# MIMUW-RL/space-gym

Measured on AMD Instinct MI355X. Metric: env-steps/sec at batch=65536, GoalContinuous3P-v0, 1/2/4/8 MI355X, higher is better.
Workload: dtype f32

## Files before the change

include/spacegym.h:

```cpp
#ifndef SPACEGYM_H
#define SPACEGYM_H

#include <stddef.h>
#include <stdint.h>

#ifdef __cplusplus
extern "C" {
#endif

#define SG_OK 0
#define SG_ERR_INVALID -1
#define SG_ERR_HIP -2
#define SG_ERR_NO_DEVICE -3

typedef struct sg_env sg_env;

typedef struct sg_config {
    char env_id[64];
    int64_t num_envs;
    uint64_t seed;
    uint32_t env_index_base;
    int32_t max_episode_steps;
    int32_t auto_reset;
    int32_t steering;
// ... 318 lines not shown
    int32_t activation;
    float log_std_min;
    float log_std_max;
    sg_policy_mlp actor;
    int32_t reserved;
} sg_squashed_policy;
int sg_squashed_act_device(sg_env *env, const sg_squashed_policy *sp, const float *obs_dev, uint64_t seed, uint64_t step,
                           int32_t deterministic, float *action_out, float *logp_out, void *hip_stream);
int sg_squashed_sample_device(sg_env *env, const sg_squashed_policy *sp, int64_t n, const float *obs, const float *eps,
                              float *action_out, float *logp_out, void *hip_stream);
typedef struct sg_squashed_grads {
    uint32_t struct_size;
    uint32_t reserved;
    sg_policy_grads_mlp actor;
} sg_squashed_grads;
int sg_squashed_grad_device(sg_env *env, const sg_squashed_policy *sp, int64_t n, const float *obs, const float *eps,
                            const float *g_action, const float *g_logp, const sg_squashed_grads *grads, void *workspace,
                            size_t workspace_bytes, void *hip_stream);
size_t sg_squashed_grad_workspace_bytes(sg_env *env, const sg_squashed_policy *sp, int64_t n);
int sg_rollout_squashed_device(sg_env *env, int32_t n_steps, const sg_squashed_policy *sp, uint64_t seed, uint64_t first_step,
                               int32_t deterministic, float *obs, float *action, float *logp, float *reward, uint8_t *done,
                               uint8_t *truncated, const sg_terminal_list *terminal_list, void *hip_stream);

int sg_vector_field(sg_env *env, const void *actions_host, const float *ship_host, float *out_host);

void *sg_host_alloc(size_t bytes);
void sg_host_free(void *ptr);

int sg_set_profiling(sg_env *env, int32_t on);
int sg_get_profile(sg_env *env, int64_t *launches, double *total_ms, double *min_ms, double *max_ms);

const char *sg_rollout_kernel(sg_env *env, int32_t n_steps);

void *sg_stream(const sg_env *env);

const char *sg_version(void);

#ifdef __cplusplus
}
#endif
#endif
```

space_gym_amd/_native.py:

```python
import ctypes as C
import os

_HERE = os.path.dirname(os.path.abspath(__file__))
LIB_PATH = os.environ.get("SPACEGYM_LIB") or os.path.join(_HERE, "lib", "libspacegym_hip.so")
_lib = None


class SgConfig(C.Structure):
    _fields_ = [("env_id", C.c_char * 64), ("num_envs", C.c_int64), ("seed", C.c_uint64),
                ("env_index_base", C.c_uint32), ("max_episode_steps", C.c_int32), ("auto_reset", C.c_int32),
                ("steering", C.c_int32)]


class SgParams(C.Structure):
    _fields_ = [("struct_size", C.c_uint32), ("n_planets", C.c_int32), ("randomize", C.c_int32), ("reserved", C.c_int32),
                ("goal_vel_reward_scale", C.c_double), ("safety_reward_scale", C.c_double), ("goal_sparse_reward", C.c_double),
                ("survival_reward_scale", C.c_double), ("danger_zone", C.c_double),
                ("ref_orbit_a", C.c_double), ("ref_orbit_eccentricity", C.c_double), ("ref_orbit_angle", C.c_double),
                ("numerator_C", C.c_double), ("rad_penalty_C", C.c_double), ("act_penalty_C", C.c_double), ("step_size", C.c_double),
                ("ship_moi", C.c_double), ("max_engine_force", C.c_double)]


class SgTerminalList(C.Structure):
    _fields_ = [("count", C.c_void_p), ("step_env", C.c_void_p), ("obs", C.c_void_p), ("capacity", C.c_uint32)]
# ... 167 lines not shown
    "sg_priority_begin_device": (C.c_int, [_vp, C.POINTER(SgPriority), _vp]),
    "sg_priority_commit_device": (C.c_int, [_vp, C.POINTER(SgPriority), C.c_int32, C.c_int32, C.c_int32, _vp]),
    "sg_priority_update_device": (C.c_int, [_vp, C.POINTER(SgPriority), C.c_int64, _vp, _vp, _vp]),
    "sg_priority_sample_config_init": (None, [C.POINTER(SgPrioritySampleConfig)]),
    "sg_priority_sample_device": (C.c_int, [_vp, C.POINTER(SgReplay), C.POINTER(SgPriority), C.POINTER(SgPrioritySampleConfig), C.c_int64,
                                            C.POINTER(SgPriorityDraw), _vp]),
    "sg_policy_act_device": (C.c_int, [_vp, C.POINTER(SgPolicy), _vp, C.c_uint64, C.c_uint64, C.c_int32, _vp, _vp, _vp, _vp]),
    "sg_rollout_policy_device": (C.c_int, [_vp, C.c_int32, C.POINTER(SgPolicy), C.c_uint64, C.c_uint64, C.c_int32, _vp, _vp, _vp, _vp,
                                           _vp, _vp, _vp, C.POINTER(SgTerminalList), _vp, _vp]),
    "sg_policy_evaluate_device": (C.c_int, [_vp, C.POINTER(SgPolicy), C.c_int64, _vp, _vp, _vp, _vp, _vp, _vp]),
    "sg_policy_grad_device": (C.c_int, [_vp, C.POINTER(SgPolicy), C.c_int64, _vp, _vp, _vp, _vp, _vp, C.POINTER(SgPolicyGrads), _vp, C.c_size_t, _vp]),
    "sg_policy_grad_workspace_bytes": (C.c_size_t, [_vp, C.POINTER(SgPolicy), C.c_int64]),
    "sg_q_evaluate_device": (C.c_int, [_vp, C.POINTER(SgQnet), C.c_int64, _vp, _vp, _vp, _vp, _vp]),
    "sg_q_grad_device": (C.c_int, [_vp, C.POINTER(SgQnet), C.c_int64, _vp, _vp, _vp, _vp, C.POINTER(SgQnetGrads), _vp, _vp, C.c_size_t, _vp]),
    "sg_q_grad_workspace_bytes": (C.c_size_t, [_vp, C.POINTER(SgQnet), C.c_int64]),
    "sg_policy_action_device": (C.c_int, [_vp, C.POINTER(SgPolicy), C.c_int64, _vp, _vp, _vp, _vp]),
    "sg_policy_action_grad_device": (C.c_int, [_vp, C.POINTER(SgPolicy), C.c_int64, _vp, _vp, _vp, C.POINTER(SgPolicyGrads), _vp, C.c_size_t, _vp]),
    "sg_squashed_act_device": (C.c_int, [_vp, C.POINTER(SgSquashedPolicy), _vp, C.c_uint64, C.c_uint64, C.c_int32, _vp, _vp, _vp]),
    "sg_squashed_sample_device": (C.c_int, [_vp, C.POINTER(SgSquashedPolicy), C.c_int64, _vp, _vp, _vp, _vp, _vp]),
    "sg_squashed_grad_device": (C.c_int, [_vp, C.POINTER(SgSquashedPolicy), C.c_int64, _vp, _vp, _vp, _vp, C.POINTER(SgSquashedGrads), _vp,
                                          C.c_size_t, _vp]),
    "sg_squashed_grad_workspace_bytes": (C.c_size_t, [_vp, C.POINTER(SgSquashedPolicy), C.c_int64]),
    "sg_rollout_squashed_device": (C.c_int, [_vp, C.c_int32, C.POINTER(SgSquashedPolicy), C.c_uint64, C.c_uint64, C.c_int32, _vp, _vp, _vp, _vp,
                                             _vp, _vp, C.POINTER(SgTerminalList), _vp]),
    "sg_get_state": (C.c_int, [_vp, _vp, _vp, _vp, _vp]),
    "sg_set_state": (C.c_int, [_vp, _vp, _vp, _vp, _vp]),
    "sg_vector_field": (C.c_int, [_vp, _vp, _vp, _vp]),
    "sg_host_alloc": (_vp, [C.c_size_t]),
    "sg_host_free": (None, [_vp]),
    "sg_set_profiling": (C.c_int, [_vp, C.c_int32]),
    "sg_get_profile": (C.c_int, [_vp, C.POINTER(C.c_int64), C.POINTER(C.c_double), C.POINTER(C.c_double), C.POINTER(C.c_double)]),
    "sg_stream": (_vp, [_vp]),
    "sg_rollout_kernel": (C.c_char_p, [_vp, C.c_int32]),
    "sg_random_actions_device": (C.c_int, [_vp, C.c_int32, C.c_uint64, C.c_uint64, _vp, _vp]),
    "sg_version": (C.c_char_p, []),
}


def load():
    global _lib
    if _lib is not None:
        return _lib
    if not os.path.exists(LIB_PATH):
        raise NativeError(f"{LIB_PATH} not found: build it with `python -m space_gym_amd.build` "
                          "(hipcc, gfx950). The engine is HIP-only; there is no CPU fallback.")
    try:
        import torch
    except ImportError:
        pass
    lib = C.CDLL(LIB_PATH)
    for name, (res, args) in SYMBOLS.items():
        try:
            fn = getattr(lib, name)
        except AttributeError:
            if not os.environ.get("SPACEGYM_LIB"):
                raise
            continue
        fn.restype, fn.argtypes = res, args
    _lib = lib
    return lib


def check(lib, handle, rc, what):
    if rc != 0:
        msg = lib.sg_last_error(handle)
        raise NativeError(f"{what} failed ({rc}): {msg.decode() if msg else ''}")
# ... 1 lines not shown
```

space_gym_amd/csrc/sg_engine.hip:

```cpp
#include <hip/hip_runtime.h>
#include <hip/hip_ext.h>

#include <algorithm>
#include <cmath>
#include <cstdarg>
#include <cstdio>
#include <cstdlib>
#include <cstring>
#include <limits>
#include <new>
#include <string>
#include <tuple>
#include <type_traits>
#include <utility>
#include <vector>

#include "../../include/spacegym.h"

#ifdef SG_STAMPS
constexpr int kStampSlots = 16, kStampWaves = 4096;
__device__ unsigned long long sg_dbg_stamps[kStampSlots * kStampWaves];
#ifdef SG_STAMPS_ACC_ONLY
#define SG_STAMP(slot)
#else
// ... 1076 lines not shown
    constexpr int D = 7 + 2 * N + 2;
    const bool have = (uint32_t)lane < n;
    const uint32_t slot = (lo + (have ? (uint32_t)lane : 0u)) % (uint32_t)kReplayCap;
    uint32_t step_lane;
    GoalEnv<N> e;
    float2 a;
    GoalReplay<N>::get(rb, slot, step_lane, e, a);
    double dXd, dYd;
    GoalReplay<N>::get_result(rb, slot, dXd, dYd);
    int hit;
    float rew;
    if constexpr (RS::kOn) rew = goal_reward<N>(rs.goal(c, wave_env0 + (int)(step_lane & 63u)), e.x, e.y, dXd, dYd, e.px, e.py, e.gx, e.gy, hit);
    else rew = goal_reward<N>(c, e.x, e.y, dXd, dYd, e.px, e.py, e.gx, e.gy, hit);
    count_hits(cnt, have && hit);
    const int t = (int)(step_lane >> 6), env = wave_env0 + (int)(step_lane & 63u);
    if (have) reward[(int64_t)t * B + env] = rew;
    if constexpr (TOBS) {
        e.x = (float)((double)e.x + dXd); e.y = (float)((double)e.y + dYd);
        float o[D];
        goal_observe<N>(c, e, o);
        term_append<D>(tl, have, t, env, o);
    }
}

template <int N, bool ACCEL, int kSpare, bool TOBS>
__global__ __launch_bounds__(kPairBlock) void goal_pair_rollout_kernel(const SgDev *__restrict__ cfg, const SgBuffers *__restrict__ bufs,
                                                                    int num_envs, int n_steps,
                                                                    const void *__restrict__ actions, float *__restrict__ obs,
                                                                    float *__restrict__ reward, uint8_t *__restrict__ done,
                                                                    uint8_t *__restrict__ truncated,
                                                                    typename std::conditional<TOBS, TermList, NoTermList>::type tl,
                                                                    int *__restrict__ status) {
#define SG_ROLLOUT_PROFILED 0
#define SG_ROLLOUT_RS
#include "sg_goal_pair_rollout.inc"
#undef SG_ROLLOUT_RS
#undef SG_ROLLOUT_PROFILED
}
template <int N, bool ACCEL, int kSpare, bool TOBS>
__global__ __launch_bounds__(kPairBlock) void goal_pair_rollout_profiled_kernel(const SgDev *__restrict__ cfg,
                                                                             const SgBuffers *__restrict__ bufs, int num_envs, int n_steps,
                                                                             const void *__restrict__ actions, float *__restrict__ obs,
                                                                             float *__restrict__ reward, uint8_t *__restrict__ done,
                                                                             uint8_t *__restrict__ truncated,
                                                                             typename std::conditional<TOBS, TermList, NoTermList>::type tl,
                                                                             int *__restrict__ status, ProfileSource rs) {
#define SG_ROLLOUT_PROFILED 1
#define SG_ROLLOUT_RS , rs
#include "sg_goal_pair_rollout.inc"
#undef SG_ROLLOUT_RS
#undef SG_ROLLOUT_PROFILED
}

template <typename F, typename... X>
__device__ __forceinline__ void pair_step(const SgDev *cfg, SgBuffers b, int num_envs, const void *actions, float *obs,
                                          float *reward, uint8_t *done, uint8_t *truncated, float *terminal_obs, X... extra) {
    __shared__ float hand[kHand * kBlock];
    const int tid = threadIdx.x & (kBlock - 1);
    const bool pilot = threadIdx.x < kBlock;
    const int i = blockIdx.x * kBlock + tid;
    const bool live = i < num_envs;
    const int ii = live ? i : 0;
    typename F::Env e;
    F::load_env(b, ii, e);
    const SgDev &c = *cfg;
    if constexpr (F::kTouchParams) {
        const uint32_t *cw = reinterpret_cast<const uint32_t *>(cfg);
        uint32_t touch = 0u;
#pragma unroll
        for (int k = 0; k < (int)(sizeof(SgDev) / 4); k += 16) touch ^= cw[k];
        touch ^= cw[sizeof(SgDev) / 4 - 1];
        asm volatile("" ::"s"(touch));
    }
    const bool discrete = c.discrete_actions != 0;
    float2 a = make_float2(0.0f, 0.0f);
    if constexpr (F::kFinishAction) load_action(discrete, actions, ii, a.x, a.y);
    float *q = hand + tid;
    if (pilot) {
        if constexpr (!F::kFinishAction) load_action(discrete, actions, ii, a.x, a.y);
        StepResult r;
        F::integrate(c, e, a, r);
        const uint64_t ux = __double_as_longlong(r.dXd), uy = __double_as_longlong(r.dYd);
        q[0 * kBlock] = __uint_as_float((uint32_t)ux); q[1 * kBlock] = __uint_as_float((uint32_t)(ux >> 32));
// ... 1569 lines not shown
    __attribute__((always_inline)) sg_env() = default;
    SgDev dev = {};
    SgDev *d_cfg = nullptr;
    SgBuffers buf = {};
    SgBuffers *d_buf = nullptr;
    int device = 0;
    int fresh = 0;
    hipStream_t stream = nullptr;
    float *d_actions = nullptr, *d_obs = nullptr, *d_reward = nullptr, *d_tobs = nullptr, *d_ship = nullptr, *d_planets = nullptr, *d_goal = nullptr;
    uint8_t *d_done = nullptr, *d_trunc = nullptr;
    int32_t *d_elapsed = nullptr;
    int *h_status = nullptr, *d_status = nullptr;
    uint8_t *d_pack = nullptr, *h_pack[2] = {};
    uint8_t *h_pack_dev[2] = {};
    int host_out = 0;
    size_t pack_bytes = 0, pack_tobs = 0, pack_reward = 0, pack_done = 0, pack_trunc = 0;
    hipEvent_t step_event = nullptr;
    int pack_cur = 0, step_pending = 0, step_tobs = 0;
    double *d_ep_ret = nullptr, *d_epo_ret = nullptr;
    int32_t *d_ep_len = nullptr, *d_epo_len = nullptr;
    size_t pack_base_bytes = 0, pack_ep_ret = 0, pack_ep_len = 0;
    int step_eps = 0;
    int last_end = -1;
    sg_normalize norm = {};
    double *d_nstate = nullptr, *d_returns = nullptr, *d_npart = nullptr, *d_nmtab = nullptr, *d_nstab = nullptr;
    uint8_t *d_nsel = nullptr;
    int32_t norm_cap = 0;
    std::vector<void *> norm_retired;
    unsigned long long *d_cnt = nullptr;
    std::vector<hipStream_t> pending;
    hipEvent_t join_event = nullptr;
    int step_kernel = 0;
    int rollout_kernel = 0;
    std::string err, kernel_name;
    char id[64] = {};
    int profiling = 0;
    int unfused_rollout = 0;
    int num_cus = 0;
    int step_wgs_per_cu = 0;
    std::vector<std::pair<hipEvent_t, hipEvent_t>> prof_events;
    sg_render_config rcfg = {};
    RenderSlot *d_rslots = nullptr;
    float2 *d_rtrace = nullptr;
    int4 *d_rprims = nullptr;
    int2 *d_rverts = nullptr;
    int32_t *d_rcounts = nullptr, *d_rids = nullptr;
    uint32_t *d_repoch = nullptr;
    uint32_t repoch = 0;
    uint8_t *d_rframes = nullptr;
    size_t rframes_bytes = 0;
    void *d_ptab = nullptr;
    uint8_t *d_pidx = nullptr;
    int n_prof = 0;
    std::vector<sg_reward_profile> prof, prof_given;
    int prof_wgs_per_cu = 0;
    int squashed_ready = 0;
    int q_ready = 0;
    int policy_grad_ready = 0;
    int policy_ready = 0;
};

static thread_local std::string g_create_error;

static int fail(sg_env *e, int code, const char *fmt, ...) {
    char msg[512];
    va_list ap;
// ... 134 lines not shown
    id[63] = 0;
    SgDev d;
    if (fill_config(id, d)) return fail(nullptr, SG_ERR_INVALID, "sg_create: unknown env id '%s'", id);
    if (params) {
        if (params->struct_size != sizeof(sg_params)) return fail(nullptr, SG_ERR_INVALID, "sg_create_ex: sg_params of %u bytes, %zu expected (sg_params_init first)", params->struct_size, sizeof(sg_params));
        if (const char *bad = apply_params(*params, d)) return fail(nullptr, SG_ERR_INVALID, "sg_create_ex: %s", bad);
    }
    d.steering_acceleration = cfg->steering == 1 ? 1 : 0;
    if (cfg->steering != 0 && cfg->steering != 1) return fail(nullptr, SG_ERR_INVALID, "sg_create: steering %d not served (0: Steering.velocity, 1: Steering.acceleration)", cfg->steering);
    if (!step_size_supported(d)) return fail(nullptr, SG_ERR_INVALID, "sg_create: step size %g not supported (the heading may advance by at most pi / 4 per env-step)", (double)d.h);
    int n_dev = 0;
    if (hipGetDeviceCount(&n_dev) != hipSuccess || n_dev <= 0)
        return fail(nullptr, SG_ERR_NO_DEVICE, "sg_create: no HIP device visible; the engine has no CPU path");
    if (device < 0 || device >= n_dev) return fail(nullptr, SG_ERR_INVALID, "sg_create: device %d out of range (%d visible)", device, n_dev);
    SG_HIP(nullptr, hipSetDevice(device));
    sg_env *e = new (std::nothrow) sg_env();
    if (!e) return fail(nullptr, SG_ERR_INVALID, "sg_create: out of host memory");
    sg_normalize_init(&e->norm); e->norm.obs = e->norm.reward = 0;
    std::memcpy(e->id, id, sizeof(id));
    d.num_envs = (int32_t)cfg->num_envs;
    d.env_index_base = cfg->env_index_base;
    d.seed_lo = (uint32_t)cfg->seed; d.seed_hi = (uint32_t)(cfg->seed >> 32);
    if (cfg->max_episode_steps > 0) d.max_episode_steps = cfg->max_episode_steps;
    d.auto_reset = cfg->auto_reset ? 1 : 0;
    e->dev = d; e->device = device; e->fresh = 1;
    e->num_cus = 256;
    (void)hipDeviceGetAttribute(&e->num_cus, hipDeviceAttributeMultiprocessorCount, device);
    const char *sw = getenv("SPACEGYM_STEP_WGS_PER_CU");
    e->step_wgs_per_cu = sw && atoi(sw) > 0 ? atoi(sw) : 2;
    const char *sk = getenv("SPACEGYM_STEP_KERNEL");
    e->step_kernel = sk ? (!strcmp(sk, "single") ? 1 : !strcmp(sk, "pair") ? 2 : 0) : 0;
    const char *rk = getenv("SPACEGYM_ROLLOUT_KERNEL");
    e->rollout_kernel = rk ? (!strcmp(rk, "single") ? 1 : !strcmp(rk, "pair") ? 2 : 0) : 0;
    const size_t B = (size_t)d.num_envs, D = (size_t)obs_dim(d);
    const size_t NP = d.family == SG_FAMILY_GOAL ? (size_t)d.n_planets : 0;
    hipError_t st = hipSuccess;
    auto ok = [&](hipError_t r) { if (st == hipSuccess) st = r; };
    ok(hipStreamCreateWithFlags(&e->stream, hipStreamNonBlocking));
    ok(hipEventCreateWithFlags(&e->join_event, hipEventDisableTiming));
    ok(hipHostMalloc((void **)&e->h_status, sizeof(int), hipHostMallocMapped));
    if (st == hipSuccess) { *e->h_status = 0; ok(hipHostGetDevicePointer((void **)&e->d_status, e->h_status, 0)); }
    ok(dmalloc(&e->d_cfg, 1));
    ok(dmalloc(&e->d_buf, 1));
    ok(dmalloc(&e->d_cnt, 4));
    ok(dmalloc(&e->buf.q0, B)); ok(dmalloc(&e->buf.q1, B));
    ok(dmalloc(&e->buf.ctr, B)); ok(dmalloc(&e->buf.aux, B));
    if (d.family == SG_FAMILY_GOAL) {
        ok(dmalloc(&e->buf.pl[0], B));
        if (d.n_planets > 2) ok(dmalloc(&e->buf.pl[1], B));
        ok(dmalloc(&e->buf.cshift, B));
        ok(dmalloc(&e->buf.epq, (size_t)kQDepth * kQCols * B));
        ok(dmalloc(&e->buf.ephi, B));
    } else if (d.randomize_orbit) {
        ok(dmalloc(&e->buf.orbd, B));
    }
    ok(dmalloc(&e->d_actions, 2 * B)); ok(dmalloc(&e->d_obs, D * B)); ok(dmalloc(&e->d_tobs, D * B));
    ok(dmalloc(&e->d_reward, B)); ok(dmalloc(&e->d_done, B)); ok(dmalloc(&e->d_trunc, B));
    ok(dmalloc(&e->d_ship, 6 * B)); ok(dmalloc(&e->d_goal, 2 * B)); ok(dmalloc(&e->d_elapsed, B));
    if (NP) ok(dmalloc(&e->d_planets, 2 * NP * B));
    {
        auto up = [](size_t x) { return (x + 15) & ~(size_t)15; };
        e->pack_tobs = up(sizeof(float) * D * B);
        e->pack_reward = e->pack_tobs + up(sizeof(float) * D * B);
        e->pack_done = e->pack_reward + up(sizeof(float) * B);
        e->pack_trunc = e->pack_done + up(B);
        e->pack_bytes = e->pack_base_bytes = e->pack_trunc + up(B);
// ... 275 lines not shown
        return;
    }
    hipEvent_t a = nullptr, b = nullptr;
    if (hipEventCreate(&a) != hipSuccess || hipEventCreate(&b) != hipSuccess) {
        kernel<<<grid, BLOCK, lds, s>>>(args...);
        return;
    }
    hipExtLaunchKernelGGL(kernel, dim3(grid), dim3(BLOCK), lds, s, a, b, 0, args...);
    e->prof_events.emplace_back(a, b);
}
template <int BLOCK = kBlock, typename K, typename... Args>
static void launch_maybe_timed(sg_env *e, K kernel, int grid, hipStream_t s, Args... args) {
    launch_maybe_timed_lds<BLOCK>(e, kernel, grid, 0, s, args...);
}

static void count_flags(sg_env *e, const uint8_t *done, const uint8_t *trunc, int64_t n_steps, hipStream_t s) {
    if (!e->buf.cnt) return;
    const int64_t n = n_steps * (int64_t)e->dev.num_envs;
    const int grid = (int)std::min<int64_t>((n + kBlock - 1) / kBlock, 1024);
    count_flags_kernel<<<grid, kBlock, 0, s>>>(done, trunc, n, e->buf.cnt);
}

enum RolloutKind {
    kRolloutSteps,
    kRolloutOneWave,
    kRolloutPair,
};
constexpr int kGoalQueueDepth = 3;
constexpr int kKeplerPairQueueDepth = 4;
struct RolloutPlan {
    RolloutKind kind;
    bool pair_step;
    int depth;
};
static RolloutPlan rollout_plan(const sg_env *e) {
    const bool kepler = e->dev.family == SG_FAMILY_KEPLER;
    RolloutPlan p = {kRolloutSteps, false, 0};
    p.pair_step = e->step_kernel ? e->step_kernel == 2 : grid_for(e) <= (kepler ? 2 : 1) * e->num_cus;
    if (e->unfused_rollout == 1) return p;
    const bool pair = e->rollout_kernel ? e->rollout_kernel == 2 : true;
    if (e->n_prof && !pair) return p;
    p.kind = pair ? kRolloutPair : kRolloutOneWave;
    p.depth = !kepler ? kGoalQueueDepth : pair ? kKeplerPairQueueDepth : 0;
    return p;
}

static size_t profile_entry_bytes(const sg_env *e) {
    return e->dev.family == SG_FAMILY_GOAL ? sizeof(GoalRewardProfile) : sizeof(KeplerRewardProfile);
}

template <bool PAIR, bool PROF, typename F>
static void select_step_kernel(const sg_env *e, F f) {
    if (e->dev.family == SG_FAMILY_GOAL) {
        select_goal(e, [&](auto np, auto acc) {
            if constexpr (PAIR && PROF) f(goal_pair_step_profiled_kernel<np, acc>);
            else if constexpr (PAIR) f(goal_pair_step_kernel<np, acc>);
            else if constexpr (PROF) f(goal_step_profiled_kernel<np, acc>);
            else f(goal_step_kernel<np, acc>);
        });
    } else {
        select_bool(needs_general_kernels(e->dev), [&](auto acc) {
            if constexpr (PAIR && PROF) f(kepler_pair_step_profiled_kernel<acc>);
            else if constexpr (PAIR) f(kepler_pair_step_kernel<acc>);
            else if constexpr (PROF) f(kepler_step_profiled_kernel<acc>);
            else f(kepler_step_kernel<acc>);
        });
    }
}

static int launch_step(sg_env *e, const void *actions, float *obs, float *reward, uint8_t *done, uint8_t *trunc,
                       float *tobs, hipStream_t s, int stream_out = 0) {
    const int grid = grid_for(e), nenv = (int)e->dev.num_envs, n_sub = (int)((e->dev.num_envs + 63) / 64);
    const bool pair = rollout_plan(e).pair_step;
    const int wgs_per_cu = e->n_prof ? std::max(1, std::min(e->step_wgs_per_cu, e->prof_wgs_per_cu)) : e->step_wgs_per_cu;
    const int tgrid = std::min(grid, wgs_per_cu * e->num_cus);
    const size_t lds = (size_t)e->n_prof * profile_entry_bytes(e);
// ... 44 lines not shown
    }
    e->prof_events.clear();
    if (launches) *launches = n;
    if (total_ms) *total_ms = tot;
    if (min_ms) *min_ms = n ? mn : 0;
    if (max_ms) *max_ms = mx;
    return SG_OK;
}

static int step_device_impl(sg_env *e, const void *actions, float *obs, float *reward, uint8_t *done, uint8_t *trunc,
                            float *tobs, double *ep_ret, int32_t *ep_len, hipStream_t s, const char *who) {
    if (!e || !actions || !obs || !reward || !done || !trunc) return e ? fail(e, SG_ERR_INVALID, "%s: null buffer", who) : SG_ERR_INVALID;
    int rc = status_error(e, who);
    if (rc) return rc;
    launch_step(e, actions, obs, reward, done, trunc, tobs, s);
    episode_pass(e, 1, reward, done, trunc, ep_ret, ep_len, 0, kNoEpList, s);
    count_flags(e, done, trunc, 1, s);
    SG_HIP(e, hipGetLastError());
    note_device_work(e, s);
    return norm_pass(e, 1, obs, reward, done, tobs, kNoTermList, s, false, who);
}

extern "C" int sg_step_device(sg_env *e, const void *actions, float *obs, float *reward, uint8_t *done, uint8_t *trunc,
                              float *tobs, void *hip_stream) {
    return step_device_impl(e, actions, obs, reward, done, trunc, tobs, nullptr, nullptr, (hipStream_t)hip_stream, "sg_step_device");
}

extern "C" int sg_step_device_episodes(sg_env *e, const void *actions, float *obs, float *reward, uint8_t *done, uint8_t *trunc,
                                       float *tobs, double *ep_ret, int32_t *ep_len, void *hip_stream) {
    if (!e) return SG_ERR_INVALID;
    if (!e->d_ep_ret) return fail(e, SG_ERR_INVALID, "sg_step_device_episodes: episode statistics are off (sg_set_episode_stats)");
    if (!ep_ret || !ep_len) return fail(e, SG_ERR_INVALID, "sg_step_device_episodes: null episode row");
    return step_device_impl(e, actions, obs, reward, done, trunc, tobs, ep_ret, ep_len, (hipStream_t)hip_stream, "sg_step_device_episodes");
}

extern "C" const char *sg_rollout_kernel(sg_env *e, int32_t ) {
    if (!e) return "";
    const RolloutPlan plan = rollout_plan(e);
    const bool kepler = e->dev.family == SG_FAMILY_KEPLER;
    const char *acc = needs_general_kernels(e->dev) ? "true" : "false", *prof = e->n_prof ? "_profiled" : "";
    const int np = e->dev.n_planets;
    char buf[96];
    if (plan.kind == kRolloutSteps) {
        const char *pair = plan.pair_step ? "_pair" : "";
        if (kepler) snprintf(buf, sizeof(buf), "kepler%s_step%s_kernel<%s>", pair, prof, acc);
        else snprintf(buf, sizeof(buf), "goal%s_step%s_kernel<%d, %s>", pair, prof, np, acc);
    } else if (plan.kind == kRolloutOneWave) {
        if (kepler) snprintf(buf, sizeof(buf), "kepler_rollout_kernel<%s>", acc);
        else snprintf(buf, sizeof(buf), "goal_rollout_kernel<%d, %s, %d>", np, acc, plan.depth);
    } else {
        if (kepler) snprintf(buf, sizeof(buf), "kepler_pair_rollout%s_kernel<%s, %d>", prof, acc, plan.depth);
        else snprintf(buf, sizeof(buf), "goal_pair_rollout%s_kernel<%d, %s, %d, false>", prof, np, acc, plan.depth);
    }
    e->kernel_name = buf;
    return e->kernel_name.c_str();
}

static int rollout_impl(sg_env *e, int32_t n_steps, const void *actions, float *obs, float *reward, uint8_t *done, uint8_t *trunc,
                        const sg_terminal_list *list, const sg_episode_list *eps, hipStream_t s, const char *who) {
    if (!e || n_steps < 0 || !actions || !obs || !reward || !done || !trunc) return e ? fail(e, SG_ERR_INVALID, "%s: bad argument", who) : SG_ERR_INVALID;
    if (list && (!list->count || !list->step_env || !list->obs)) return fail(e, SG_ERR_INVALID, "%s: incomplete terminal list", who);
    if (eps && (!eps->count || !eps->step_env || !eps->ret || !eps->length || !eps->truncated))
        return fail(e, SG_ERR_INVALID, "%s: incomplete episode list", who);
    int rc = status_error(e, who);
    if (rc) return rc;
    if (e->d_nstate && e->norm.update) {
        rc = norm_reserve(e, n_steps, s, who);
        if (rc) return rc;
    }
    TermList tl = {nullptr, nullptr, nullptr, 0u};
    if (list) {
        tl.count = list->count; tl.step_env = list->step_env; tl.obs = list->obs; tl.capacity = list->capacity;
        SG_HIP(e, hipMemsetAsync(tl.count, 0, sizeof(uint32_t), s));
    }
    EpList el = kNoEpList;
    if (eps) {
        el.count = eps->count; el.step_env = eps->step_env; el.ret = eps->ret; el.length = eps->length;
        el.truncated = eps->truncated; el.capacity = eps->capacity;
        SG_HIP(e, hipMemsetAsync(el.count, 0, sizeof(uint32_t), s));
    }
    if (n_steps == 0) return SG_OK;
    const int grid = grid_for(e);
    const void *a2 = actions;
    const size_t action_bytes = e->dev.discrete_actions ? sizeof(int32_t) : 2 * sizeof(float);
    const bool acc = needs_general_kernels(e->dev);
    const int nenv = e->dev.num_envs;
    const RolloutPlan plan = rollout_plan(e);
    const bool kepler = e->dev.family == SG_FAMILY_KEPLER;
    const int K = (int)n_steps;
    const ProfileSource ps = {e->d_ptab, e->d_pidx};
    if (plan.kind == kRolloutPair && kepler) {
        select_bool(acc, [&](auto ac) {
            if (e->n_prof) launch_maybe_timed<kPairBlock>(e, kepler_pair_rollout_profiled_kernel<ac, kKeplerPairQueueDepth>, grid, s, e->d_cfg, e->buf, K, a2, obs, reward, done, trunc, tl, e->d_status, ps);
            else launch_maybe_timed<kPairBlock>(e, kepler_pair_rollout_kernel<ac, kKeplerPairQueueDepth>, grid, s, e->d_cfg, e->buf, K, a2, obs, reward, done, trunc, tl, e->d_status);
        });
    } else if (plan.kind == kRolloutOneWave && kepler) {
        select_bool(acc, [&](auto ac) { launch_maybe_timed(e, kepler_rollout_kernel<ac>, grid, s, e->d_cfg, e->buf, K, a2, obs, reward, done, trunc, tl); });
    } else if (plan.kind == kRolloutPair) {
        auto launch = [&](auto tobs, auto tlist) {
            select_goal(e, [&](auto np, auto ac) {
                if (e->n_prof) launch_maybe_timed<kPairBlock>(e, goal_pair_rollout_profiled_kernel<np, ac, kGoalQueueDepth, tobs>, grid, s, e->d_cfg, e->d_buf, nenv, K, a2, obs, reward, done, trunc, tlist, e->d_status, ps);
                else launch_maybe_timed<kPairBlock>(e, goal_pair_rollout_kernel<np, ac, kGoalQueueDepth, tobs>, grid, s, e->d_cfg, e->d_buf, nenv, K, a2, obs, reward, done, trunc, tlist, e->d_status);
            });
        };
        if (list) launch(std::true_type{}, tl);
        else launch(std::false_type{}, NoTermList());
    } else if (plan.kind == kRolloutOneWave) {
        select_goal(e, [&](auto np, auto ac) {
            launch_maybe_timed(e, goal_rollout_kernel<np, ac, kGoalQueueDepth>, grid, s, e->d_cfg, e->buf, K, a2, obs, reward, done, trunc, tl);
        });
    } else {
        const size_t B = (size_t)e->dev.num_envs, D = (size_t)obs_dim(e->dev);
        for (int32_t t = 0; t < n_steps; t++) {
            launch_step(e, (const char *)actions + t * action_bytes * B, obs + t * D * B, reward + t * B, done + t * B, trunc + t * B,
                        list ? e->d_tobs : nullptr, s, 1);
            if (list && e->dev.auto_reset)
                term_compact_kernel<<<grid, kBlock, 0, s>>>(e->d_cfg, done + t * B, e->d_tobs, (int)t, (int)D, tl);
        }
    }
    episode_pass(e, n_steps, reward, done, trunc, nullptr, nullptr, 0, el, s);
    count_flags(e, done, trunc, n_steps, s);
    SG_HIP(e, hipGetLastError());
    note_device_work(e, s);
    return norm_pass(e, n_steps, obs, reward, done, nullptr, tl, s, false, who);
}

extern "C" int sg_rollout_device(sg_env *e, int32_t n_steps, const void *actions, float *obs, float *reward,
                                 uint8_t *done, uint8_t *trunc, void *hip_stream) {
    return rollout_impl(e, n_steps, actions, obs, reward, done, trunc, nullptr, nullptr, (hipStream_t)hip_stream, "sg_rollout_device");
}

extern "C" int sg_rollout_device_terminal(sg_env *e, int32_t n_steps, const void *actions, float *obs, float *reward,
// ... 2196 lines not shown
```

space_gym_amd/csrc/sg_goal_pair_rollout.inc:

```

    const SgBuffers &b = *bufs;
    using Spare = SpareEpisode<N>;
    using Queue = EpisodeQueue<N>;
    using Integ = Integrator<N, N, true, ACCEL>;
    using Replay = GoalReplay<N>;
    __shared__ float spare[kSpare * Spare::kFields * kBlock];
    __shared__ float ring[kRing * kHand * kBlock];
    __shared__ float rbuf[(kBlock / 64) * Replay::kWords * kReplayCap];
    __shared__ uint32_t spare_hi[kBlock];
    __shared__ uint32_t handed[kBlock / 64], taken[kBlock / 64];
    __shared__ uint32_t rp_tail[kBlock / 64];
    __shared__ uint32_t rp_claim[kBlock / 64], rp_done[kBlock / 64];
    constexpr int D = 7 + 2 * N + 2;
    SG_REAL(0);
    const int tid = threadIdx.x & (kBlock - 1), pair = tid >> 6, lane = tid & 63;
    const bool pilot = threadIdx.x < kBlock;
    const int i = blockIdx.x * kBlock + tid;
    const bool live = i < num_envs;
    const int ii = live ? i : 0;
    const int64_t B = num_envs;
    GoalEnv<N> e;
    load_goal_env<N>(b, ii, e);
    uint2 ct = b.ctr[ii];
    const SgDev &c = *cfg;
    {
        const uint32_t *cw = reinterpret_cast<const uint32_t *>(cfg);
        uint32_t touch = 0u;
#pragma unroll
        for (int k = 0; k < (int)(sizeof(SgDev) / 4); k += 16) touch ^= cw[k];
        touch ^= cw[sizeof(SgDev) / 4 - 1];
        asm volatile("" ::"s"(touch));
    }
    const bool discrete = c.discrete_actions != 0;
    float *const rb = rbuf + pair * Replay::kWords * kReplayCap;
    if (!pilot) spare_hi[tid] = ct.y;
    if (threadIdx.x < kBlock / 64) { handed[threadIdx.x] = 0u; taken[threadIdx.x] = 0u; rp_tail[threadIdx.x] = 0u; rp_claim[threadIdx.x] = 0u; rp_done[threadIdx.x] = 0u; }
    __syncthreads();
    SG_REAL(1);

    if (pilot) {
        SG_ACC_DECL;
        __builtin_amdgcn_s_setprio(3);
        const bool hand_over = c.auto_reset && live;
        const bool auto_reset = c.auto_reset != 0;
        StepConsts kc = step_consts(c);
        asm volatile("" : "+v"(kc.max_engine_force), "+v"(kc.h), "+v"(kc.half_world), "+v"(kc.gm), "+v"(kc.omega_limit), "+v"(kc.planet_r),
                          "+v"(kc.max_thruster_force), "+v"(kc.inv_moi), "+v"(kc.planet_r_d));
        int max_steps = c.max_episode_steps;
        asm volatile("" : "+v"(max_steps));
        float2 a_next = load_action_raw(discrete, actions, ii);
        uint32_t taken_seen = 0u;
        uint32_t head = 0u, tail_seen = 0u;
        for (int t = 0; t < n_steps; t++) {
            const float2 a = decode_action(discrete, a_next);
            if (t + 1 < n_steps) a_next = load_action_raw(discrete, actions, (int64_t)(t + 1) * B + ii);
            if (t - (int)taken_seen >= kRing && !wait_flag<SG_PILOT_SLEEP>(&taken[pair], (uint32_t)(t - kRing + 1), &taken_seen)) { *status = 1; break; }
            if (head + 64u - tail_seen > (uint32_t)kReplayCap) tail_seen = lds_flag_load_uniform(&rp_tail[pair]);
            const bool defer = hand_over && head + 64u - tail_seen <= (uint32_t)kReplayCap;

            const int slot = t % kRing;
            StepResult r;
            int rk;
            {
                Integ I;
                SG_ACC(0);
                goal_env_begin<N, ACCEL>(kc, e, a.x, a.y, I);
                SG_ACC(1);
                rk = I.run(r, [&]() __attribute__((always_inline)) -> bool { return defer; });
                SG_ACC_ADD(7, __any(r.done) ? 1 : 0);
                SG_ACC_ADD(10, __any(r.path == kPathScipyErr || r.path == kPathScipyClear) ? 1 : 0);
                SG_ACC_ADD(11, __any((r.path == kPathScipyErr || r.path == kPathScipyClear) && r.n_rk > 1) ? 1 : 0);
                SG_ACC(2);
            }
            const bool replayed = rk == kRkEventDeferred;
            uint32_t rslot = 0u;
            {
                const unsigned long long dm = __ballot(replayed);
                if (dm) {
                    rslot = (head + (uint32_t)__popcll(dm & ((1ull << lane) - 1ull))) % (uint32_t)kReplayCap;
                    if (replayed) Replay::put(rb, rslot, ((uint32_t)t << 6) | (uint32_t)lane, e, a);
                    head += (uint32_t)__popcll(dm);
                }
            }
            e.x = (float)((double)e.x + r.dXd); e.y = (float)((double)e.y + r.dYd); e.vx = r.vx; e.vy = r.vy; e.om = r.om;
            e.th = wrap_two_pi(e.th + r.dth);
            SG_ACC(3);
            SG_ACC(4);
            {
                float *q = ring + (slot * kHand) * kBlock + tid;
                const uint64_t ux = __double_as_longlong(r.dXd), uy = __double_as_longlong(r.dYd);
                q[0 * kBlock] = __uint_as_float((uint32_t)ux); q[1 * kBlock] = __uint_as_float((uint32_t)(ux >> 32));
                q[2 * kBlock] = __uint_as_float((uint32_t)uy); q[3 * kBlock] = __uint_as_float((uint32_t)(uy >> 32));
                q[4 * kBlock] = e.th; q[5 * kBlock] = e.vx; q[6 * kBlock] = e.vy; q[7 * kBlock] = e.om;
                q[8 * kBlock] = __uint_as_float((uint32_t)r.done | (replayed ? 2u | (rslot << 8) : 0u));
            }
            lds_flag_store(&handed[pair], (uint32_t)(t + 1));
            SG_ACC(5);
            const uint32_t el = ct.x + 1u;
            const int trunc = !r.done && (int)el >= max_steps;
            const bool restart = live && (r.done | trunc) && auto_reset;
            if (live) ct.x = el;
            if (restart) {
                const uint32_t k = ct.y + 1u;
                if ((int32_t)(lds_flag_load(&spare_hi[tid]) - k) >= 0) {
                    const float *q = spare + ((int)(k % (uint32_t)kSpare) * Spare::kFields) * kBlock + tid;
                    e.x = q[0 * kBlock]; e.y = q[1 * kBlock]; e.th = q[2 * kBlock]; e.vx = q[3 * kBlock];
                    e.vy = q[4 * kBlock]; e.om = q[5 * kBlock];
#pragma unroll
                    for (int j = 0; j < N; j++) { e.px[j] = q[(8 + 2 * j) * kBlock]; e.py[j] = q[(9 + 2 * j) * kBlock]; }
                } else {
                    Tiling T;
                    T.episode = k;
                    ShipInit s;
                    float gx, gy;
                    goal_reset<N>(c, c.env_index_base + (uint32_t)i, T, s, e.px, e.py, gx, gy);
                    e.x = s.x; e.y = s.y; e.th = s.th; e.vx = s.vx; e.vy = s.vy; e.om = s.om;
                }
                ct = make_uint2(0u, k);
            }
            SG_ACC(8);
        }
        SG_ACC_WRITE(blockIdx.x * 8 + pair);
        SG_REAL(2);
        if (live) {
            b.q0[i] = make_float4(e.x, e.y, e.th, e.vx);
            reinterpret_cast<float2 *>(b.q1 + i)[0] = make_float2(e.vy, e.om);
            store_goal_planets<N>(b, i, e);
            b.ctr[i] = ct;
        }
        {
            uint32_t lo = 0u;
            if (lane == 0) lo = atomicMax(&rp_claim[pair], head);
            lo = (uint32_t)__builtin_amdgcn_readfirstlane((int)lo);
            __builtin_amdgcn_fence(__ATOMIC_SEQ_CST, "wavefront");
#pragma unroll 1
            while ((int32_t)(head - lo) > 0) {
                const uint32_t n = min(head - lo, 64u);
                goal_replay_integrate<N, ACCEL>(c, rb, lo, n, lane);
                lo += n;
            }
            lds_flag_store(&rp_done[pair], 1u);
        }
        SG_REAL(3);
        return;
    }

    SG_ACC_DECL;
    const bool auto_reset = c.auto_reset != 0;
    const int wave_env0 = i - lane;
    unsigned long long *const cnt = b.cnt;
    GoalStepConsts fc = goal_step_consts(c);
#if SG_ROLLOUT_PROFILED
    {
        const GoalRewardView v = rs.goal(c, ii);
        fc.danger_r2 = v.danger_r2; fc.survival = v.survival; fc.goal_scale = v.goal_scale; fc.safety_scale = v.safety_scale;
        fc.sparse = v.sparse;
    }
#endif
    asm volatile("" : "+v"(fc.goal_r2), "+v"(fc.danger_r2), "+v"(fc.survival), "+v"(fc.goal_scale), "+v"(fc.safety_scale),
                      "+v"(fc.sparse), "+v"(fc.planet_r), "+v"(fc.two_over_world));
    int max_steps = c.max_episode_steps;
    asm volatile("" : "+v"(max_steps));
    uint32_t hi = ct.y;
    uint4 aux = b.aux[ii];
    float4 cs = b.cshift[ii];
    if (auto_reset) {
        const uint32_t q_hi = b.ephi[ii];
        const int n_have = live ? min(max((int32_t)(q_hi - ct.y), 0), kSpare) : 0;
        float4 rec[kSpare][kQCols];
#pragma unroll
        for (int s = 0; s < kSpare; s++)
            if (s < n_have) {
                const float4 *p = Queue::slot(b.epq, B, i, ct.y + 1u + (uint32_t)s);
#pragma unroll
                for (int col = 0; col < kQCols; col++)
                    if (col != 3 || N > 2) rec[s][col] = p[(uint32_t)col * (uint32_t)B];
            }
#pragma unroll
        for (int s = 0; s < kSpare; s++)
            if (s < n_have) Spare::put_record(spare, (int)((ct.y + 1u + (uint32_t)s) % (uint32_t)kSpare), tid, rec[s]);
        hi = ct.y + (uint32_t)n_have;
        lds_flag_store(&spare_hi[tid], hi);
    }
    auto refill = [&]() {
        SG_ACC_ADD(10, 1);
        if (live && hi - ct.y < (uint32_t)kSpare) {
            Tiling T;
            T.episode = hi + 1u;
            ShipInit s;
            float px[N], py[N], gx, gy;
            goal_reset<N>(c, c.env_index_base + (uint32_t)i, T, s, px, py, gx, gy);
            Spare::put(spare, (int)(T.episode % (uint32_t)kSpare), tid, s, px, py, gx, gy, T);
            Queue::put(b.epq, B, i, s, px, py, gx, gy, T);
            hi = T.episode;
            lds_flag_store(&spare_hi[tid], hi);
        }
    };
    constexpr uint32_t kKeep = 1u;
    if (auto_reset && __any(live && hi - ct.y < kKeep)) refill();
    uint32_t tail = 0u, complete = 0u;
    bool mine = true;
    typedef __attribute__((address_space(1))) float gfloat;
    typedef __attribute__((address_space(1))) uint8_t gbyte;
    gfloat *obs_p = (gfloat *)obs + (int64_t)ii * D, *rew_p = (gfloat *)reward + ii;
    gbyte *done_p = (gbyte *)done + ii, *trunc_p = (gbyte *)truncated + ii;
    asm volatile("" : "+v"(obs_p), "+v"(rew_p), "+v"(done_p), "+v"(trunc_p));
    for (int t = 0; t < n_steps; t++) {
        SG_ACC(0);
        if (!wait_flag(&handed[pair], (uint32_t)(t + 1))) { *status = 2; break; }
        SG_ACC(1);
        double dXd, dYd;
        float th, vx, vy, om;
        int dn;
        bool replayed;
        {
            const int slot = t % kRing;
            const float *q = ring + (slot * kHand) * kBlock + tid;
            const uint64_t ux = (uint64_t)__float_as_uint(q[0 * kBlock]) | ((uint64_t)__float_as_uint(q[1 * kBlock]) << 32);
            const uint64_t uy = (uint64_t)__float_as_uint(q[2 * kBlock]) | ((uint64_t)__float_as_uint(q[3 * kBlock]) << 32);
            dXd = __longlong_as_double((long long)ux); dYd = __longlong_as_double((long long)uy);
            th = q[4 * kBlock]; vx = q[5 * kBlock]; vy = q[6 * kBlock]; om = q[7 * kBlock];
            const uint32_t w8 = __float_as_uint(q[8 * kBlock]);
            dn = (int)(w8 & 1u);
            replayed = (w8 & 2u) != 0u;
            if (replayed) Replay::put_goal(rb, w8 >> 8, e.gx, e.gy);
            complete += (uint32_t)__popcll(__ballot(replayed));
        }
        lds_flag_store(&taken[pair], (uint32_t)(t + 1));
        SG_ACC(3);
        float o[D], r;
        int hit;
        r = goal_reward<N>(fc, e.x, e.y, dXd, dYd, e.px, e.py, e.gx, e.gy, hit);
        count_hits(cnt, live && hit && !replayed);
        e.x = (float)((double)e.x + dXd); e.y = (float)((double)e.y + dYd); e.vx = vx; e.vy = vy; e.om = om; e.th = th;
        const uint32_t el = ct.x + 1u;
        const int trunc = !dn && (int)el >= max_steps;
        const int fin = dn | trunc;
        const bool restart = live && fin && auto_reset;
        if (live) ct.x = el;
        SG_ACC(4);
        if constexpr (TOBS) {
            if (__any(restart && !replayed)) {
                goal_observe<N>(fc, e, o);
                term_append<D>(tl, restart && !replayed, t, i, o);
            }
        }
        const uint32_t keep = t + 1 < n_steps ? kKeep : 0u;
        if (auto_reset && __any(live && hi - ct.y < (restart ? keep + 1u : keep))) refill();
        SG_ACC(6);
        if (restart) {
            ct = make_uint2(0u, ct.y + 1u);
            Spare::get(spare, (int)(ct.y % (uint32_t)kSpare), tid, e, aux, cs);
        }
        SG_ACC(12);
        goal_observe<N>(fc, e, o);
// ... 55 lines not shown
```

space_gym_amd/vector_env.py:

```python
import ctypes as C

import numpy as np

from . import _native
from .registration import (ENV_CLASSES, ENV_SPECS, constructor_kwargs, is_discrete, obs_dim, single_action_space,
                           single_observation_space)
from .spaces import MultiDiscrete, batch_box


_KEEP = object()


class StepInfo(dict):
    """Batched info: {"TimeLimit.truncated": bool[B], "terminal_observation": float32[B, D] (rows of finished envs)}; with
    episode statistics on also "episode": {"r": float64[B], "l": int32[B]} and the mask "_episode": bool[B] of the envs whose
    episode ended (gymnasium's vector convention; other rows of "r" / "l" read NaN / -1).
    A per-env list of dicts (old gym VectorEnv) would cost more than the step itself at B = 65536."""


RENDER_SIZES = (16, 2048)
RENDER_CAPACITY = 16


REWARD_PROFILES_MAX = 256
# ... 1825 lines not shown
        draw_out = gather_out = None
        if out is not None:
            missing = [k for k in ("index", "cell", "weight") if k not in out]
            if missing:
                raise ValueError(f"out: {', '.join(missing)} missing (index, cell and weight are required; leaf, discount, steps optional)")
            draw_out = {k: out[k] for k in ("index", "cell", "weight", "leaf") if k in out}
            gather_out = {k: v for k, v in out.items() if k not in ("cell", "weight", "leaf")}
        d = self.replay_priority_draw_torch(ring, prio, n, seed=seed, beta=beta, stratified=stratified, out=draw_out)
        batch = self.replay_sample_torch(ring, n, seed=seed, n_step=n_step, gamma=gamma, index=d["index"], out=gather_out)
        if int(n) > 0 and normalize:
            d["weight"].div_(d["weight"].max())
        if out is not None:
            return out
        batch["index"], batch["cell"], batch["weight"] = d["index"], d["cell"], d["weight"]
        return batch

    def random_actions_torch(self, n_steps, seed=0, first_step=0, out=None):
        import torch
        shape = (int(n_steps), self.num_envs) if self.discrete else (int(n_steps), self.num_envs, 2)
        if out is None:
            out = torch.empty(shape, dtype=torch.int32 if self.discrete else torch.float32, device=f"cuda:{self.device}")
        assert tuple(out.shape) == shape and out.is_contiguous()
        rc = self._lib.sg_random_actions_device(self._h, int(n_steps), C.c_uint64(seed), C.c_uint64(first_step),
                                                C.c_void_p(out.data_ptr()), self._stream())
        self._ck(rc, "sg_random_actions_device")
        return out

    def set_unfused_rollout(self, on):
        self._ck(self._lib.sg_set_unfused_rollout(self._h, int(on)), "sg_set_unfused_rollout")

    def rollout_kernel(self, n_steps):
        return self._lib.sg_rollout_kernel(self._h, int(n_steps)).decode()

    def set_profiling(self, on):
        self._ck(self._lib.sg_set_profiling(self._h, int(bool(on))), "sg_set_profiling")

    def get_profile(self):
        n, tot, mn, mx = C.c_int64(), C.c_double(), C.c_double(), C.c_double()
        self._ck(self._lib.sg_get_profile(self._h, C.byref(n), C.byref(tot), C.byref(mn), C.byref(mx)), "sg_get_profile")
        return n.value, tot.value, mn.value, mx.value


_ENGINE_KWARGS = ("device", "seed", "env_index_base", "max_episode_steps", "auto_reset", "validate_actions", "terminal_observation",
                  "copy", "steering", "env_kwargs", "from_class", "episode_statistics", "normalize_obs", "normalize_reward",
                  "norm_gamma", "norm_epsilon", "clip_obs", "clip_reward", "render", "reward_profiles")
_NORM_KWARGS = ("normalize_obs", "normalize_reward", "norm_gamma", "norm_epsilon", "clip_obs", "clip_reward")


class DeviceSnapshot:
    __slots__ = ("buffer", "num_envs", "env_id")

    def __init__(self, buffer, num_envs, env_id):
        self.buffer, self.num_envs, self.env_id = buffer, int(num_envs), env_id


def make_vec(env_id, num_envs=1, **kwargs):
    devices = kwargs.pop("devices", None)
    if devices is not None:
        from .multi_device import MultiDeviceVectorEnv
        return MultiDeviceVectorEnv(env_id, num_envs, devices, **kwargs)
    engine = {k: kwargs.pop(k) for k in list(kwargs) if k in _ENGINE_KWARGS}
    if kwargs:
        engine["env_kwargs"] = {**(engine.get("env_kwargs") or {}), **kwargs}
    return SpaceGymVectorEnv(env_id, num_envs, **engine)


# ... 6 lines not shown
```

Before: 30.12 billion.

## Add specialized pair rollout kernel with compile-time constants and wide LDS ring

Adds a specialized goal pair rollout kernel used when envs are block-aligned, auto-reset is on, no counters or profiling, and no general kernels are needed. It turns liveness, discrete-action, auto-reset and hit-counter checks into compile-time constants, and packs the pilot-to-worker LDS ring handoff into 64-bit stores and loads instead of separate 32-bit words. This is meant to cut branches, register pressure and LDS instruction count in the hot loop. The cost is another set of kernel instantiations, and the new path depends on aligned may_alias LDS accesses being correct.

New measurement: 30.11 billion. About the same (-0.0%).

```diff
diff --git a/include/spacegym.h b/include/spacegym.h
--- a/include/spacegym.h
+++ b/include/spacegym.h
@@ -374,6 +374,8 @@
 
 const char *sg_rollout_kernel(sg_env *env, int32_t n_steps);
 
+const char *sg_rollout_variant(sg_env *env);
+
 void *sg_stream(const sg_env *env);
 
 const char *sg_version(void);
diff --git a/space_gym_amd/_native.py b/space_gym_amd/_native.py
--- a/space_gym_amd/_native.py
+++ b/space_gym_amd/_native.py
@@ -223,6 +223,7 @@
     "sg_get_profile": (C.c_int, [_vp, C.POINTER(C.c_int64), C.POINTER(C.c_double), C.POINTER(C.c_double), C.POINTER(C.c_double)]),
     "sg_stream": (_vp, [_vp]),
     "sg_rollout_kernel": (C.c_char_p, [_vp, C.c_int32]),
+    "sg_rollout_variant": (C.c_char_p, [_vp]),
     "sg_random_actions_device": (C.c_int, [_vp, C.c_int32, C.c_uint64, C.c_uint64, _vp, _vp]),
     "sg_version": (C.c_char_p, []),
 }
diff --git a/space_gym_amd/csrc/sg_engine.hip b/space_gym_amd/csrc/sg_engine.hip
--- a/space_gym_amd/csrc/sg_engine.hip
+++ b/space_gym_amd/csrc/sg_engine.hip
@@ -1132,9 +1132,11 @@
                                                                     typename std::conditional<TOBS, TermList, NoTermList>::type tl,
                                                                     int *__restrict__ status) {
 #define SG_ROLLOUT_PROFILED 0
+#define SG_ROLLOUT_SPECIAL 0
 #define SG_ROLLOUT_RS
 #include "sg_goal_pair_rollout.inc"
 #undef SG_ROLLOUT_RS
+#undef SG_ROLLOUT_SPECIAL
 #undef SG_ROLLOUT_PROFILED
 }
 template <int N, bool ACCEL, int kSpare, bool TOBS>
@@ -1146,9 +1148,31 @@
                                                                              typename std::conditional<TOBS, TermList, NoTermList>::type tl,
                                                                              int *__restrict__ status, ProfileSource rs) {
 #define SG_ROLLOUT_PROFILED 1
+#define SG_ROLLOUT_SPECIAL 0
 #define SG_ROLLOUT_RS , rs
 #include "sg_goal_pair_rollout.inc"
 #undef SG_ROLLOUT_RS
+#undef SG_ROLLOUT_SPECIAL
+#undef SG_ROLLOUT_PROFILED
+}
+#ifndef SG_ROLLOUT_WIDE_RING
+#define SG_ROLLOUT_WIDE_RING 1
+#endif
+template <int N, int kSpare, bool TOBS, bool DISCRETE>
+__global__ __launch_bounds__(kPairBlock) void goal_pair_full_rollout_kernel(const SgDev *__restrict__ cfg, const SgBuffers *__restrict__ bufs,
+                                                                         int num_envs, int n_steps,
+                                                                         const void *__restrict__ actions, float *__restrict__ obs,
+                                                                         float *__restrict__ reward, uint8_t *__restrict__ done,
+                                                                         uint8_t *__restrict__ truncated,
+                                                                         typename std::conditional<TOBS, TermList, NoTermList>::type tl,
+                                                                         int *__restrict__ status) {
+    constexpr bool ACCEL = false;
+#define SG_ROLLOUT_PROFILED 0
+#define SG_ROLLOUT_SPECIAL 1
+#define SG_ROLLOUT_RS
+#include "sg_goal_pair_rollout.inc"
+#undef SG_ROLLOUT_RS
+#undef SG_ROLLOUT_SPECIAL
 #undef SG_ROLLOUT_PROFILED
 }
 
@@ -2784,6 +2808,7 @@
     hipEvent_t join_event = nullptr;
     int step_kernel = 0;
     int rollout_kernel = 0;
+    int rollout_specialize = 1;
     std::string err, kernel_name;
     char id[64] = {};
     int profiling = 0;
@@ -2984,6 +3009,8 @@
     e->step_kernel = sk ? (!strcmp(sk, "single") ? 1 : !strcmp(sk, "pair") ? 2 : 0) : 0;
     const char *rk = getenv("SPACEGYM_ROLLOUT_KERNEL");
     e->rollout_kernel = rk ? (!strcmp(rk, "single") ? 1 : !strcmp(rk, "pair") ? 2 : 0) : 0;
+    const char *rsp = getenv("SPACEGYM_ROLLOUT_SPECIALIZE");
+    e->rollout_specialize = rsp && !strcmp(rsp, "0") ? 0 : 1;
     const size_t B = (size_t)d.num_envs, D = (size_t)obs_dim(d);
     const size_t NP = d.family == SG_FAMILY_GOAL ? (size_t)d.n_planets : 0;
     hipError_t st = hipSuccess;
@@ -3325,16 +3352,19 @@
     RolloutKind kind;
     bool pair_step;
     int depth;
+    bool full;
 };
 static RolloutPlan rollout_plan(const sg_env *e) {
     const bool kepler = e->dev.family == SG_FAMILY_KEPLER;
-    RolloutPlan p = {kRolloutSteps, false, 0};
+    RolloutPlan p = {kRolloutSteps, false, 0, false};
     p.pair_step = e->step_kernel ? e->step_kernel == 2 : grid_for(e) <= (kepler ? 2 : 1) * e->num_cus;
     if (e->unfused_rollout == 1) return p;
     const bool pair = e->rollout_kernel ? e->rollout_kernel == 2 : true;
     if (e->n_prof && !pair) return p;
     p.kind = pair ? kRolloutPair : kRolloutOneWave;
     p.depth = !kepler ? kGoalQueueDepth : pair ? kKeplerPairQueueDepth : 0;
+    p.full = pair && !kepler && e->rollout_specialize && e->dev.num_envs % kBlock == 0 && e->dev.auto_reset && !e->buf.cnt &&
+             !e->n_prof && !needs_general_kernels(e->dev);
     return p;
 }
 
@@ -3445,6 +3475,11 @@
     if (!e->d_ep_ret) return fail(e, SG_ERR_INVALID, "sg_step_device_episodes: episode statistics are off (sg_set_episode_stats)");
     if (!ep_ret || !ep_len) return fail(e, SG_ERR_INVALID, "sg_step_device_episodes: null episode row");
     return step_device_impl(e, actions, obs, reward, done, trunc, tobs, ep_ret, ep_len, (hipStream_t)hip_stream, "sg_step_device_episodes");
+}
+
+extern "C" const char *sg_rollout_variant(sg_env *e) {
+    if (!e) return "";
+    return rollout_plan(e).full ? "full" : "general";
 }
 
 extern "C" const char *sg_rollout_kernel(sg_env *e, int32_t ) {
@@ -3511,6 +3546,14 @@
         select_bool(acc, [&](auto ac) { launch_maybe_timed(e, kepler_rollout_kernel<ac>, grid, s, e->d_cfg, e->buf, K, a2, obs, reward, done, trunc, tl); });
     } else if (plan.kind == kRolloutPair) {
         auto launch = [&](auto tobs, auto tlist) {
+            if (plan.full) {
+                select_planets(e->dev.n_planets, [&](auto np) {
+                    select_bool(e->dev.discrete_actions != 0, [&](auto disc) {
+                        launch_maybe_timed<kPairBlock>(e, goal_pair_full_rollout_kernel<np, kGoalQueueDepth, tobs, disc>, grid, s, e->d_cfg, e->d_buf, nenv, K, a2, obs, reward, done, trunc, tlist, e->d_status);
+                    });
+                });
+                return;
+            }
             select_goal(e, [&](auto np, auto ac) {
                 if (e->n_prof) launch_maybe_timed<kPairBlock>(e, goal_pair_rollout_profiled_kernel<np, ac, kGoalQueueDepth, tobs>, grid, s, e->d_cfg, e->d_buf, nenv, K, a2, obs, reward, done, trunc, tlist, e->d_status, ps);
                 else launch_maybe_timed<kPairBlock>(e, goal_pair_rollout_kernel<np, ac, kGoalQueueDepth, tobs>, grid, s, e->d_cfg, e->d_buf, nenv, K, a2, obs, reward, done, trunc, tlist, e->d_status);
diff --git a/space_gym_amd/csrc/sg_goal_pair_rollout.inc b/space_gym_amd/csrc/sg_goal_pair_rollout.inc
--- a/space_gym_amd/csrc/sg_goal_pair_rollout.inc
+++ b/space_gym_amd/csrc/sg_goal_pair_rollout.inc
@@ -5,7 +5,13 @@
     using Integ = Integrator<N, N, true, ACCEL>;
     using Replay = GoalReplay<N>;
     __shared__ float spare[kSpare * Spare::kFields * kBlock];
+#if SG_ROLLOUT_SPECIAL && SG_ROLLOUT_WIDE_RING
+    __shared__ __attribute__((aligned(8))) float ring[kRing * kHand * kBlock];
+    typedef double __attribute__((may_alias)) ring_f64;
+    typedef float2 __attribute__((may_alias)) ring_f32x2;
+#else
     __shared__ float ring[kRing * kHand * kBlock];
+#endif
     __shared__ float rbuf[(kBlock / 64) * Replay::kWords * kReplayCap];
     __shared__ uint32_t spare_hi[kBlock];
     __shared__ uint32_t handed[kBlock / 64], taken[kBlock / 64];
@@ -16,8 +22,13 @@
     const int tid = threadIdx.x & (kBlock - 1), pair = tid >> 6, lane = tid & 63;
     const bool pilot = threadIdx.x < kBlock;
     const int i = blockIdx.x * kBlock + tid;
+#if SG_ROLLOUT_SPECIAL
+    constexpr bool live = true;
+    const int ii = i;
+#else
     const bool live = i < num_envs;
     const int ii = live ? i : 0;
+#endif
     const int64_t B = num_envs;
     GoalEnv<N> e;
     load_goal_env<N>(b, ii, e);
@@ -31,7 +42,11 @@
         touch ^= cw[sizeof(SgDev) / 4 - 1];
         asm volatile("" ::"s"(touch));
     }
+#if SG_ROLLOUT_SPECIAL
+    constexpr bool discrete = DISCRETE;
+#else
     const bool discrete = c.discrete_actions != 0;
+#endif
     float *const rb = rbuf + pair * Replay::kWords * kReplayCap;
     if (!pilot) spare_hi[tid] = ct.y;
     if (threadIdx.x < kBlock / 64) { handed[threadIdx.x] = 0u; taken[threadIdx.x] = 0u; rp_tail[threadIdx.x] = 0u; rp_claim[threadIdx.x] = 0u; rp_done[threadIdx.x] = 0u; }
@@ -41,8 +56,12 @@
     if (pilot) {
         SG_ACC_DECL;
         __builtin_amdgcn_s_setprio(3);
+#if SG_ROLLOUT_SPECIAL
+        constexpr bool hand_over = true, auto_reset = true;
+#else
         const bool hand_over = c.auto_reset && live;
         const bool auto_reset = c.auto_reset != 0;
+#endif
         StepConsts kc = step_consts(c);
         asm volatile("" : "+v"(kc.max_engine_force), "+v"(kc.h), "+v"(kc.half_world), "+v"(kc.gm), "+v"(kc.omega_limit), "+v"(kc.planet_r),
                           "+v"(kc.max_thruster_force), "+v"(kc.inv_moi), "+v"(kc.planet_r_d));
@@ -87,12 +106,20 @@
             SG_ACC(3);
             SG_ACC(4);
             {
+#if SG_ROLLOUT_SPECIAL && SG_ROLLOUT_WIDE_RING
+                float *q = ring + (slot * kHand) * kBlock;
+                reinterpret_cast<ring_f64 *>(q)[tid] = r.dXd; reinterpret_cast<ring_f64 *>(q)[kBlock + tid] = r.dYd;
+                reinterpret_cast<ring_f32x2 *>(q)[2 * kBlock + tid] = make_float2(e.th, e.vx);
+                reinterpret_cast<ring_f32x2 *>(q)[3 * kBlock + tid] = make_float2(e.vy, e.om);
+                q[8 * kBlock + tid] = __uint_as_float((uint32_t)r.done | (replayed ? 2u | (rslot << 8) : 0u));
+#else
                 float *q = ring + (slot * kHand) * kBlock + tid;
                 const uint64_t ux = __double_as_longlong(r.dXd), uy = __double_as_longlong(r.dYd);
                 q[0 * kBlock] = __uint_as_float((uint32_t)ux); q[1 * kBlock] = __uint_as_float((uint32_t)(ux >> 32));
                 q[2 * kBlock] = __uint_as_float((uint32_t)uy); q[3 * kBlock] = __uint_as_float((uint32_t)(uy >> 32));
                 q[4 * kBlock] = e.th; q[5 * kBlock] = e.vx; q[6 * kBlock] = e.vy; q[7 * kBlock] = e.om;
                 q[8 * kBlock] = __uint_as_float((uint32_t)r.done | (replayed ? 2u | (rslot << 8) : 0u));
+#endif
             }
             lds_flag_store(&handed[pair], (uint32_t)(t + 1));
             SG_ACC(5);
@@ -146,9 +173,17 @@
     }
 
     SG_ACC_DECL;
+#if SG_ROLLOUT_SPECIAL
+    constexpr bool auto_reset = true;
+#else
     const bool auto_reset = c.auto_reset != 0;
+#endif
     const int wave_env0 = i - lane;
+#if SG_ROLLOUT_SPECIAL
+    constexpr unsigned long long *cnt = nullptr;
+#else
     unsigned long long *const cnt = b.cnt;
+#endif
     GoalStepConsts fc = goal_step_consts(c);
 #if SG_ROLLOUT_PROFILED
     {
@@ -215,12 +250,20 @@
         bool replayed;
         {
             const int slot = t % kRing;
+#if SG_ROLLOUT_SPECIAL && SG_ROLLOUT_WIDE_RING
+            const float *q = ring + (slot * kHand) * kBlock;
+            dXd = reinterpret_cast<const ring_f64 *>(q)[tid]; dYd = reinterpret_cast<const ring_f64 *>(q)[kBlock + tid];
+            const float2 tv = reinterpret_cast<const ring_f32x2 *>(q)[2 * kBlock + tid], vo = reinterpret_cast<const ring_f32x2 *>(q)[3 * kBlock + tid];
+            th = tv.x; vx = tv.y; vy = vo.x; om = vo.y;
+            const uint32_t w8 = __float_as_uint(q[8 * kBlock + tid]);
+#else
             const float *q = ring + (slot * kHand) * kBlock + tid;
             const uint64_t ux = (uint64_t)__float_as_uint(q[0 * kBlock]) | ((uint64_t)__float_as_uint(q[1 * kBlock]) << 32);
             const uint64_t uy = (uint64_t)__float_as_uint(q[2 * kBlock]) | ((uint64_t)__float_as_uint(q[3 * kBlock]) << 32);
             dXd = __longlong_as_double((long long)ux); dYd = __longlong_as_double((long long)uy);
             th = q[4 * kBlock]; vx = q[5 * kBlock]; vy = q[6 * kBlock]; om = q[7 * kBlock];
             const uint32_t w8 = __float_as_uint(q[8 * kBlock]);
+#endif
             dn = (int)(w8 & 1u);
             replayed = (w8 & 2u) != 0u;
             if (replayed) Replay::put_goal(rb, w8 >> 8, e.gx, e.gy);
diff --git a/space_gym_amd/vector_env.py b/space_gym_amd/vector_env.py
--- a/space_gym_amd/vector_env.py
+++ b/space_gym_amd/vector_env.py
@@ -1881,6 +1881,9 @@
     def rollout_kernel(self, n_steps):
         return self._lib.sg_rollout_kernel(self._h, int(n_steps)).decode()
 
+    def rollout_variant(self):
+        return self._lib.sg_rollout_variant(self._h).decode()
+
     def set_profiling(self, on):
         self._ck(self._lib.sg_set_profiling(self._h, int(bool(on))), "sg_set_profiling")
 
```
